# ytgui/SPT-proto

Measured on NVIDIA B200. Metric: sparse_mha_fwd_bwd_tokens_per_s, higher is better.
Workload: dtype bf16

## Files before the change

### spt_proto_b200/csrc/attn_common.cuh

```cuda
#pragma once
#include <cstdlib>
#include <cstring>

#include "tc.cuh"

namespace spt {
namespace attn_tc {

using namespace tc;

constexpr int BM = 128;
constexpr int BN = 64;
constexpr int STAGES = 3;
constexpr int N_MATH = 256;
constexpr int THREADS = 320;
template <int D>
struct Dim {
    static_assert(D == 64 || D == 128, "head dim must be 64 or 128");
    static constexpr int NSUB = D / 64;
    static constexpr int OWN_SUB = BM * 64 * 2, T_SUB = BN * 64 * 2;
    static constexpr int OWN_BYTES = NSUB * OWN_SUB, T_BYTES = NSUB * T_SUB;
    static constexpr int TMEM_COLS = D == 64 ? 256 : 512;
    static constexpr int CTAS = D == 64 ? 2 : 1;
    static constexpr int FWD_SMEM = OWN_BYTES + 2 * STAGES * T_BYTES + 1024  + 1024  + 256 ;
// ... 221 lines not shown
                d0, d1);
            if (CLAMP) {
                d0 = in0 ? d0 : 0.0f;
                d1 = in1 ? d1 : 0.0f;
            }
            pe[i >> 1] = pack_bf16(e0, e1) & m;
            pd[i >> 1] = pack_bf16(d0, d1) & m;
        }
    }
}

#ifdef SPT_ATTN_PROF
static __device__ unsigned long long g_prof[3][16];
struct Prof {
    long long t[8] = {0, 0, 0, 0, 0, 0, 0, 0};
    long long last;
    __device__ __forceinline__ void start() { last = clock64(); }
    __device__ __forceinline__ void lap(int slot) {
        const long long now = clock64();
        t[slot] += now - last;
        last = now;
    }
    __device__ __forceinline__ void flush(int kernel, int base, bool on) {
        if (on)
            for (int i = 0; i < 8; ++i) atomicAdd(&g_prof[kernel][base + i], (unsigned long long)t[i]);
    }
};
#define PROF(...) __VA_ARGS__
#else
#define PROF(...)
#endif

struct Smem {
    uint32_t base;
    unsigned char *ptr;
};
__device__ __forceinline__ Smem align_smem(unsigned char *raw) {
    const uint32_t a = smem_u32(raw);
    const uint32_t base = (a + 1023) & ~1023u;
    return {base, raw + (base - a)};
}
__device__ __forceinline__ void math_warps_sync() { asm volatile("bar.sync 1, %0;" ::"n"(N_MATH) : "memory"); }

__device__ __forceinline__ void store_row32(__nv_bfloat16 *dst, const uint32_t (&r)[32], float s) {
#pragma unroll
    for (int i = 0; i < 32; i += 8) {
        float t[8];
#pragma unroll
        for (int u = 0; u < 8; ++u) t[u] = __uint_as_float(r[i + u]) * s;
        Vec16<__nv_bfloat16>::store(dst + i, t);
    }
}

}

namespace attn_tc128 {
int launch_bwd_kv128(const CUtensorMap &mq, const CUtensorMap &mk, const CUtensorMap &mv, const CUtensorMap &md,
                     const uint32_t *mask, const int32_t *extra0, const float *ndelta, __nv_bfloat16 *gk,
                     __nv_bfloat16 *gv, int B, int S, int H, float scale, float clamp, cudaStream_t st);
int launch_bwd_q128(const CUtensorMap &mq, const CUtensorMap &mk, const CUtensorMap &mv, const CUtensorMap &md,
                    const uint32_t *mask, const int32_t *extra0, const float *ndelta, __nv_bfloat16 *gq, int B, int S,
                    int H, float scale, float clamp, cudaStream_t st);
int launch_bwd_fused128(const CUtensorMap &mq, const CUtensorMap &mk, const CUtensorMap &mv, const CUtensorMap &md,
                        const uint32_t *mask, const int32_t *extra0, const float *ndelta, float *dq_acc,
                        __nv_bfloat16 *gq, __nv_bfloat16 *gk, __nv_bfloat16 *gv, int B, int S, int H, float scale,
                        float clamp, cudaStream_t st);
int launch_fwd128(const CUtensorMap &mq, const CUtensorMap &mk, const CUtensorMap &mv, const uint32_t *mask,
                  const int32_t *extra0, __nv_bfloat16 *y, float *zsum, int B, int S, int H, float scale, float clamp,
                  int y_transposed, cudaStream_t st);
int read_prof(unsigned long long *out48, int reset);
}
}
```

### spt_proto_b200/csrc/attn_tc.cu

```cuda
#include <mutex>

#include "attn_common.cuh"

namespace spt {
namespace attn_tc {


template <int D>
__global__ void __launch_bounds__(THREADS, Dim<D>::CTAS)
attn_fwd_tc_kernel(const __grid_constant__ CUtensorMap map_q, const __grid_constant__ CUtensorMap map_k,
                   const __grid_constant__ CUtensorMap map_v, const uint32_t *__restrict__ mask,
                   const int32_t *__restrict__ extra0, __nv_bfloat16 *__restrict__ y, float *__restrict__ zsum, int S,
                   int H, float scale_log2, float clamp_log2, int y_transposed) {
    constexpr int OWN_BYTES = Dim<D>::OWN_BYTES, T_BYTES = Dim<D>::T_BYTES, OWN_SUB = Dim<D>::OWN_SUB, T_SUB = Dim<D>::T_SUB,
                  TMEM_COLS = Dim<D>::TMEM_COLS;
    constexpr int NBUF = 3;
    extern __shared__ unsigned char smem_raw[];
    const Smem sm = align_smem(smem_raw);
    const uint32_t s_q = sm.base, s_k = s_q + OWN_BYTES, s_v = s_k + STAGES * T_BYTES;
    float *s_part = reinterpret_cast<float *>(sm.ptr + OWN_BYTES + 2 * STAGES * T_BYTES);
    uint64_t *bars = reinterpret_cast<uint64_t *>(sm.ptr + OWN_BYTES + 2 * STAGES * T_BYTES + 1024);
    const uint32_t bar0 = smem_u32(bars);
    const uint32_t q_full = bar0, o_full = bar0 + 8;
    auto k_full = [&](int s) { return bar0 + 16 + s * 8; };
// ... 587 lines not shown
            const bool clamp = warp_needs_clamp(r, mk.thr);
            uint32_t pe[8], pd[8];
#define SPT_KV_HALF(OFF)                                                                                                   \
            if (key0) {                                                                                                    \
                if (clamp) bwdkv_chunk16<true, true, OFF, 32>(r, g, mrow, s_ndelta, s_ex0, c0 + OFF, shl, mk, pe, pd);     \
                else bwdkv_chunk16<true, false, OFF, 32>(r, g, mrow, s_ndelta, s_ex0, c0 + OFF, shl, mk, pe, pd);          \
            } else {                                                                                                       \
                if (clamp) bwdkv_chunk16<false, true, OFF, 32>(r, g, mrow, s_ndelta, s_ex0, c0 + OFF, shl, mk, pe, pd);    \
                else bwdkv_chunk16<false, false, OFF, 32>(r, g, mrow, s_ndelta, s_ex0, c0 + OFF, shl, mk, pe, pd);         \
            }                                                                                                              \
            tmem_st8(col + (OFF) / 2, pe);                          \
            tmem_st8(col + 32 + (OFF) / 2, pd);
            SPT_KV_HALF(0)
            SPT_KV_HALF(16)
#undef SPT_KV_HALF
            PROF(pf.lap(2);)
            tmem_st_wait();
            fence_before_sync();
            mbar_arrive(p_full(h));
            PROF(pf.lap(3);)
        }
        PROF(pf.t[5] = clock64() - t0; pf.t[4] = n_tiles; pf.flush(2, 0, threadIdx.x == 0);)
        mbar_wait(acc_full, 0);
        fence_after_sync();
        const size_t off = (((size_t)hn * S + n0 + kk) * H + hh) * D + half * (D / 2);
#pragma unroll
        for (int c = 0; c < D / 64; ++c) {
            uint32_t r[32];
            tmem_ld32(lane_base + COL_DV + half * (D / 2) + c * 32, r);
            store_row32(dv + off + c * 32, r, 1.0f);
            tmem_ld32(lane_base + COL_DK + half * (D / 2) + c * 32, r);
            store_row32(dk + off + c * 32, r, scale);
        }
    }
    fence_before_sync();
    __syncthreads();
    if (warp == 9) tmem_dealloc<TMEM_COLS>(tmem_base);
}

static int make_map(CUtensorMap *map, const void *base, int N, int S, int H, int D) {
    EncodeTiledFn fn = encode_fn();
    if (!fn) return fail(SPT_ERR_CUDA, "sparse_attn: cuTensorMapEncodeTiled entry point not available");
    cuuint64_t dims[4] = {(cuuint64_t)D, (cuuint64_t)H, (cuuint64_t)S, (cuuint64_t)N};
    cuuint64_t strides[3] = {(cuuint64_t)D * 2, (cuuint64_t)H * D * 2, (cuuint64_t)S * H * D * 2};
    cuuint32_t box[4] = {64, 1, (cuuint32_t)BN, 1};
    cuuint32_t estr[4] = {1, 1, 1, 1};
    CUresult r = fn(map, CU_TENSOR_MAP_DATA_TYPE_BFLOAT16, 4, const_cast<void *>(base), dims, strides, box, estr,
                    CU_TENSOR_MAP_INTERLEAVE_NONE, CU_TENSOR_MAP_SWIZZLE_128B, CU_TENSOR_MAP_L2_PROMOTION_L2_256B,
                    CU_TENSOR_MAP_FLOAT_OOB_FILL_NONE);
    if (r != CUDA_SUCCESS) return fail(SPT_ERR_CUDA, "sparse_attn: cuTensorMapEncodeTiled failed (%d)", (int)r);
    return SPT_OK;
}

static bool tile128() {
    static const bool on = [] { const char *e = getenv("SPT_ATTN_TILE"); return !(e && atoi(e) == 64); }();
    return on;
}
static bool bwd_fused() {
    static const bool on = [] { const char *e = getenv("SPT_ATTN_BWD_FUSED"); return e && atoi(e) == 1; }();
    return on;
}
static bool bwd_two_streams() {
    static const bool on = [] { const char *e = getenv("SPT_ATTN_BWD_STREAMS"); return !(e && atoi(e) == 0); }();
    return on;
}
struct SideStream {
    cudaStream_t stream = nullptr;
    cudaEvent_t fork = nullptr, join = nullptr;
};
static std::mutex g_side_mu;
static SideStream *side_stream(cudaStream_t caller) {
    static SideStream table[64];
    int dev = 0;
    if (cudaGetDevice(&dev) != cudaSuccess || dev < 0 || dev >= 64) return nullptr;
    SideStream &s = table[dev];
    if (!s.stream) {
        cudaStreamCaptureStatus cap = cudaStreamCaptureStatusNone;
        if (cudaStreamIsCapturing(caller, &cap) != cudaSuccess || cap != cudaStreamCaptureStatusNone) return nullptr;
        if (cudaStreamCreateWithFlags(&s.stream, cudaStreamNonBlocking) != cudaSuccess) return nullptr;
        if (cudaEventCreateWithFlags(&s.fork, cudaEventDisableTiming) != cudaSuccess ||
            cudaEventCreateWithFlags(&s.join, cudaEventDisableTiming) != cudaSuccess) {
            s.stream = nullptr;
            return nullptr;
        }
    }
    return &s;
}
static bool fwd128() {
    static const bool on = [] { const char *e = getenv("SPT_ATTN_FWD128"); return e && atoi(e) == 1; }();
    return on;
}

template <int D>
static int launch_fwd(const CUtensorMap &mq, const CUtensorMap &mk, const CUtensorMap &mv, const uint32_t *mask,
                      const int32_t *extra0, __nv_bfloat16 *y, float *zsum, int B, int S, int H, float scale, float clamp,
                      int y_transposed, cudaStream_t st) {
    if (D == 64 && fwd128()) return attn_tc128::launch_fwd128(mq, mk, mv, mask, extra0, y, zsum, B, S, H, scale, clamp, y_transposed, st);
    static const int extra_smem = [] { const char *e = getenv("SPT_ATTN_EXTRA_SMEM"); return e ? atoi(e) : 0; }();
    cudaFuncSetAttribute(attn_fwd_tc_kernel<D>, cudaFuncAttributeMaxDynamicSharedMemorySize, Dim<D>::FWD_SMEM + extra_smem);
    attn_fwd_tc_kernel<D><<<dim3(B, S / BM), THREADS, Dim<D>::FWD_SMEM + extra_smem, st>>>(mq, mk, mv, mask, extra0, y, zsum, S, H,
                                                                              scale * LOG2E, clamp * LOG2E, y_transposed);
    return after_launch("attn_fwd_tc_kernel");
}

template <int D>
static int launch_prep(const __nv_bfloat16 *y, const __nv_bfloat16 *grad_y, const float *zsum, float *delta,
// ... 146 lines not shown
```

### spt_proto_b200/csrc/attn_tc128.cu

```cuda
#include "attn_common.cuh"

namespace spt {
namespace attn_tc128 {

using namespace tc;
using namespace attn_tc;

constexpr int T = 128;
constexpr int MATH_WARPS = 16;
constexpr int THREADS = (MATH_WARPS + 2) * 32;
constexpr int W_TMA = MATH_WARPS, W_MMA = MATH_WARPS + 1;
constexpr int D = 64;
constexpr int TILE = T * D * 2;
constexpr int ST = 3;

__device__ __forceinline__ int sched_item(int round, int n_items) {
    const int G = gridDim.x;
#ifdef SPT_SCHED_PLAIN
    const int item = round * G + (int)blockIdx.x;
#else
    const int item = round * G + ((round & 1) ? G - 1 - (int)blockIdx.x : (int)blockIdx.x);
#endif
    return item < n_items ? item : -1;
}

__device__ __forceinline__ void warp_arrive(uint32_t bar, int lane) {
    fence_before_sync();
    __syncwarp();
    if (lane == 0) mbar_arrive(bar);
}


constexpr int MT = T + 4;
constexpr int ROWQ = MT * 16 + T * 4 + T * 4;
constexpr int KV_SMEM = 4 * TILE + 2 * ST * TILE + ST * ROWQ + 256 + 1024;

__global__ void __launch_bounds__(THREADS, 1)
attn_bwd_kv128_kernel(const __grid_constant__ CUtensorMap map_q, const __grid_constant__ CUtensorMap map_k,
                      const __grid_constant__ CUtensorMap map_v, const __grid_constant__ CUtensorMap map_dys,
                      const uint32_t *__restrict__ mask, const int32_t *__restrict__ extra0,
                      const float *__restrict__ ndelta, __nv_bfloat16 *__restrict__ dk, __nv_bfloat16 *__restrict__ dv,
                      int S, int H, int B, float scale, float scale_log2, float clamp_log2) {
    extern __shared__ unsigned char smem_raw[];
    const Smem sm = align_smem(smem_raw);
    const uint32_t s_k = sm.base, s_v = s_k + 2 * TILE, s_q = s_v + 2 * TILE, s_dy = s_q + ST * TILE;
    unsigned char *rowq = sm.ptr + 4 * TILE + 2 * ST * TILE;
    uint64_t *bars = reinterpret_cast<uint64_t *>(rowq + ST * ROWQ);
    const uint32_t bar0 = smem_u32(bars);
    auto own_full = [&](int i) { return bar0 + i * 8; };
    auto own_empty = [&](int i) { return bar0 + 16 + i * 8; };
    auto qd_full = [&](int s) { return bar0 + 32 + s * 8; };
    auto qd_empty = [&](int s) { return bar0 + 32 + (ST + s) * 8; };
    const uint32_t sc_full = bar0 + 32 + 2 * ST * 8, s_read = sc_full + 8, p_full = sc_full + 16, e_free = sc_full + 24,
                   acc_full = sc_full + 32, acc_empty = sc_full + 40;
    uint32_t *tmem_slot = reinterpret_cast<uint32_t *>(bars + 4 + 2 * ST + 6);

    const int warp = threadIdx.x >> 5, lane = threadIdx.x & 31;
    const int n_own = S / T;
    const int n_items = n_own * B;
    const int words = S / 32;

    if (threadIdx.x == 0) {
        for (int i = 0; i < 2; ++i) {
            mbar_init(own_full(i), 1);
            mbar_init(own_empty(i), 1);
        }
        for (int s = 0; s < ST; ++s) {
            mbar_init(qd_full(s), 2);
            mbar_init(qd_empty(s), 1);
        }
        mbar_init(sc_full, 1);
        mbar_init(s_read, MATH_WARPS);
        mbar_init(p_full, MATH_WARPS);
        mbar_init(e_free, 1);
        mbar_init(acc_full, 1);
        mbar_init(acc_empty, MATH_WARPS);
        mbar_fence_init();
    }
    if (warp == W_MMA) tmem_alloc<512>(smem_u32(tmem_slot));
    fence_before_sync();
    __syncthreads();
    fence_after_sync();
    const uint32_t tmem_base = *tmem_slot;
    constexpr uint32_t COL_S = 0, COL_DP = 128, COL_E = 256, COL_DS = 320, COL_DV = 384, COL_DK = 448;

    if (warp == W_TMA) {
        int g = 0, w = 0;
        for (int item; (item = sched_item(w, n_items)) >= 0; ++w) {
            const int kt = item / B, b = item % B;
            const int hn = b / H, hh = b % H, n0 = kt * T, n_tiles = n_own - kt;
            const size_t head = (size_t)b * S;
            const int buf = w & 1;
            if (lane == 0) {
                mbar_wait(own_empty(buf), ((w >> 1) & 1) ^ 1);
                mbar_expect_tx(own_full(buf), 2 * TILE);
                tma_owner<D>(s_k + buf * TILE, &map_k, own_full(buf), hh, n0, hn);
                tma_owner<D>(s_v + buf * TILE, &map_v, own_full(buf), hh, n0, hn);
            }
            uint4 mw[4];
#pragma unroll
            for (int u = 0; u < 4; ++u)
                mw[u] = __ldg(reinterpret_cast<const uint4 *>(mask + (head + n0 + lane + 32 * u) * words) + kt);
            for (int j = 0; j < n_tiles; ++j, ++g) {
                const int st = g % ST;
                const int r0 = (kt + j) * T;
                unsigned char *slot = rowq + st * ROWQ;
                mbar_wait(qd_empty(st), ((g / ST) & 1) ^ 1);
                if (lane == 0) {
                    mbar_expect_tx(qd_full(st), 2 * TILE + 2 * T * 4);
                    tma_owner<D>(s_q + st * TILE, &map_q, qd_full(st), hh, r0, hn);
                    tma_owner<D>(s_dy + st * TILE, &map_dys, qd_full(st), hh, r0, hn);
                    bulk_load_1d(smem_u32(slot + MT * 16), ndelta + head + r0, T * 4, qd_full(st));
                    bulk_load_1d(smem_u32(slot + MT * 16 + T * 4), extra0 + head + r0, T * 4, qd_full(st));
                }
                uint32_t *mt = reinterpret_cast<uint32_t *>(slot);
#pragma unroll
                for (int u = 0; u < 4; ++u) {
                    const int rr = lane + 32 * u;
                    mt[rr] = mw[u].x;
                    mt[MT + rr] = mw[u].y;
                    mt[2 * MT + rr] = mw[u].z;
                    mt[3 * MT + rr] = mw[u].w;
                }
                if (j + 1 < n_tiles) {
#pragma unroll
                    for (int u = 0; u < 4; ++u)
                        mw[u] = __ldg(reinterpret_cast<const uint4 *>(mask + (head + r0 + T + lane + 32 * u) * words) + kt);
                }
                __syncwarp();
                if (lane == 0) mbar_arrive(qd_full(st));
            }
        }
    } else if (warp == W_MMA) {
        constexpr uint32_t id_s = idesc_bf16(T, T, 0, 0);
        constexpr uint32_t id_a = idesc_bf16(T, D, 0, 1);
        const uint64_t dk0 = desc_kmajor(s_k, 0), dv0 = desc_kmajor(s_v, 0), dq0 = desc_kmajor(s_q, 0),
                       ddy0 = desc_kmajor(s_dy, 0), dqt0 = desc_mnmajor(s_q, 0, TILE), ddyt0 = desc_mnmajor(s_dy, 0, TILE);
        int g = 0, w = 0;
        PROF(Prof pf; pf.start(); const long long t0 = pf.last;)
        for (int item; (item = sched_item(w, n_items)) >= 0; ++w) {
            const int kt = item / B, n_tiles = n_own - kt;
            const int buf = w & 1;
            const uint64_t own_off = (uint64_t)((buf * TILE) >> 4);
            auto issue_scores = [&](int gg) {
                const int st = gg % ST;
                mbar_wait(qd_full(st), (gg / ST) & 1);
                if (gg > 0) mbar_wait(s_read, (gg - 1) & 1);
                fence_after_sync();
                if (elect_one()) {
                    const uint64_t off = (uint64_t)((st * TILE) >> 4);
#pragma unroll
                    for (int k = 0; k < D / 16; ++k) {
                        umma_bf16(tmem_base + COL_S, dk0 + own_off + k * KMAJOR_K16, dq0 + off + k * KMAJOR_K16, id_s, k != 0);
                        umma_bf16(tmem_base + COL_DP, dv0 + own_off + k * KMAJOR_K16, ddy0 + off + k * KMAJOR_K16, id_s, k != 0);
                    }
                    umma_commit(sc_full);
                }
                __syncwarp();
            };
            mbar_wait(own_full(buf), (w >> 1) & 1);
            issue_scores(g);
            for (int j = 0; j < n_tiles; ++j, ++g) {
                PROF(pf.lap(2);)
                if (j + 1 < n_tiles) issue_scores(g + 1);
                PROF(pf.lap(0);)
                const int st = g % ST;
                mbar_wait(p_full, g & 1);
                if (j == 0 && w > 0) mbar_wait(acc_empty, (w - 1) & 1);
                PROF(pf.lap(1);)
                fence_after_sync();
                if (elect_one()) {
                    const uint64_t off = (uint64_t)((st * TILE) >> 4);
#pragma unroll
                    for (int k = 0; k < T / 16; ++k) {
                        umma_bf16_ts(tmem_base + COL_DV, tmem_base + COL_E + k * 8, ddyt0 + off + k * MNMAJOR_K16, id_a, (j | k) != 0);
                        umma_bf16_ts(tmem_base + COL_DK, tmem_base + COL_DS + k * 8, dqt0 + off + k * MNMAJOR_K16, id_a, (j | k) != 0);
                    }
                    umma_commit(qd_empty(st));
                    umma_commit(e_free);
                    if (j + 1 == n_tiles) {
                        umma_commit(acc_full);
                        umma_commit(own_empty(buf));
                    }
                }
                __syncwarp();
            }
        }
        PROF(pf.t[3] = clock64() - t0; pf.t[4] = g; pf.flush(2, 8, lane == 0);)
    } else {
        const int quarter = warp & 3, cg = warp >> 2;
        const int kk = quarter * 32 + lane;
        const int wsel = kk & 3;
        const int shl = 31 - (kk >> 2);
        const MathK mk = make_math(scale_log2, clamp_log2);
        const uint32_t lane_base = tmem_base + ((uint32_t)(quarter * 32) << 16);
        const int c0 = cg * 32;
        int g = 0, w = 0;
        PROF(Prof pf; pf.start(); const long long t0 = pf.last;)
        for (int item; (item = sched_item(w, n_items)) >= 0; ++w) {
            const int kt = item / B, b = item % B;
            const int hn = b / H, hh = b % H, n0 = kt * T, n_tiles = n_own - kt;
            const bool key0 = (n0 + kk) == 0;
            for (int j = 0; j < n_tiles; ++j, ++g) {
                const int st = g % ST;
                const unsigned char *slot = rowq + st * ROWQ;
                const uint32_t *mrow = reinterpret_cast<const uint32_t *>(slot) + wsel * MT;
                const float *s_nd = reinterpret_cast<const float *>(slot + MT * 16);
                const int32_t *s_ex0 = reinterpret_cast<const int32_t *>(slot + MT * 16 + T * 4);
                mbar_wait(qd_full(st), (g / ST) & 1);
                mbar_wait(sc_full, g & 1);
                PROF(pf.lap(0);)
                fence_after_sync();
                uint32_t r[32], gr[32];
                tmem_ld32_nowait(lane_base + COL_S + c0, r);
                tmem_ld32_nowait(lane_base + COL_DP + c0, gr);
                tmem_ld_wait();
                warp_arrive(s_read, lane);
                PROF(pf.lap(1);)
                const bool clamp = warp_needs_clamp(r, mk.thr);
                bool pad = false;
                if (key0) {
#pragma unroll
                    for (int i = 0; i < 32; i += 4) {
                        const int4 e4 = *reinterpret_cast<const int4 *>(s_ex0 + c0 + i);
                        pad |= (e4.x | e4.y | e4.z | e4.w) != 0;
                    }
                }
                uint32_t pe0[8], pd0[8], pe1[8], pd1[8];
#define SPT_KV_HALF(OFF, PE, PD)                                                                                           \
                if (pad) {                                                                                                \
                    if (clamp) bwdkv_chunk16<true, true, OFF, 32>(r, gr, mrow, s_nd, s_ex0, c0 + OFF, shl, mk, PE, PD);    \
                    else bwdkv_chunk16<true, false, OFF, 32>(r, gr, mrow, s_nd, s_ex0, c0 + OFF, shl, mk, PE, PD);         \
                } else {                                                                                                   \
                    if (clamp) bwdkv_chunk16<false, true, OFF, 32>(r, gr, mrow, s_nd, s_ex0, c0 + OFF, shl, mk, PE, PD);   \
                    else bwdkv_chunk16<false, false, OFF, 32>(r, gr, mrow, s_nd, s_ex0, c0 + OFF, shl, mk, PE, PD);        \
                }
                SPT_KV_HALF(0, pe0, pd0)
                SPT_KV_HALF(16, pe1, pd1)
#undef SPT_KV_HALF
                PROF(pf.lap(2);)
                if (g > 0) {
                    mbar_wait(e_free, (g - 1) & 1);
                    fence_after_sync();
                }
                tmem_st8(lane_base + COL_E + c0 / 2, pe0);
                tmem_st8(lane_base + COL_E + c0 / 2 + 8, pe1);
                tmem_st8(lane_base + COL_DS + c0 / 2, pd0);
                tmem_st8(lane_base + COL_DS + c0 / 2 + 8, pd1);
                tmem_st_wait();
                warp_arrive(p_full, lane);
                PROF(pf.lap(3);)
            }
            mbar_wait(acc_full, w & 1);
            fence_after_sync();
            {
                uint32_t o[32];
                tmem_ld32(lane_base + COL_DV + c0, o);
                warp_arrive(acc_empty, lane);
                const size_t off = (((size_t)hn * S + n0 + kk) * H + hh) * D + (cg & 1) * 32;
                store_row32((cg < 2 ? dv : dk) + off, o, cg < 2 ? 1.0f : scale);
            }
            PROF(pf.lap(5);)
        }
        PROF(pf.t[6] = clock64() - t0; pf.t[4] = g; pf.flush(2, 0, threadIdx.x == 0);)
    }
    fence_before_sync();
    __syncthreads();
    if (warp == W_MMA) tmem_dealloc<512>(tmem_base);
}

int launch_bwd_kv128(const CUtensorMap &mq, const CUtensorMap &mk, const CUtensorMap &mv, const CUtensorMap &md,
                     const uint32_t *mask, const int32_t *extra0, const float *ndelta, __nv_bfloat16 *gk,
                     __nv_bfloat16 *gv, int B, int S, int H, float scale, float clamp, cudaStream_t st) {
    cudaFuncSetAttribute(attn_bwd_kv128_kernel, cudaFuncAttributeMaxDynamicSharedMemorySize, KV_SMEM);
    const int n_items = (S / T) * B;
    const int grid = n_items < num_sms() ? n_items : num_sms();
    attn_bwd_kv128_kernel<<<grid, THREADS, KV_SMEM, st>>>(mq, mk, mv, md, mask, extra0, ndelta, gk, gv, S, H, B, scale,
                                                        scale * LOG2E, clamp * LOG2E);
    return after_launch("attn_bwd_kv128_kernel");
}


__device__ __forceinline__ void store_row16(__nv_bfloat16 *dst, const uint32_t (&r)[16], float s) {
#pragma unroll
    for (int i = 0; i < 16; i += 8) {
        float t[8];
#pragma unroll
        for (int u = 0; u < 8; ++u) t[u] = __uint_as_float(r[i + u]) * s;
        Vec16<__nv_bfloat16>::store(dst + i, t);
    }
}
__device__ __forceinline__ void tmem_ld16(uint32_t taddr, uint32_t (&r)[16]) {
    tmem_ld16_nowait(taddr, r);
    tmem_ld_wait();
}
__device__ __forceinline__ void math_sync() { asm volatile("bar.sync 1, %0;" ::"n"(MATH_WARPS * 32) : "memory"); }

constexpr int FUSED_SMEM = 3 * TILE + 2 * ST * TILE + 2 * TILE + 2 * TILE + ST * ROWQ + 256 + 1024;
static_assert(FUSED_SMEM <= 227 * 1024, "fused backward: shared memory budget");

__global__ void __launch_bounds__(THREADS, 1)
attn_bwd_fused128_kernel(const __grid_constant__ CUtensorMap map_q, const __grid_constant__ CUtensorMap map_k,
                         const __grid_constant__ CUtensorMap map_v, const __grid_constant__ CUtensorMap map_dys,
                         const uint32_t *__restrict__ mask, const int32_t *__restrict__ extra0,
                         const float *__restrict__ ndelta, float *__restrict__ dq_acc, __nv_bfloat16 *__restrict__ dk,
                         __nv_bfloat16 *__restrict__ dv, int S, int H, int B, float scale, float scale_log2,
                         float clamp_log2) {
    extern __shared__ unsigned char smem_raw[];
    const Smem sm = align_smem(smem_raw);
    const uint32_t s_k = sm.base, s_v = s_k + 2 * TILE, s_q = s_v + TILE, s_dy = s_q + ST * TILE, s_ds = s_dy + ST * TILE,
                   s_st = s_ds + 2 * TILE;
    unsigned char *rowq = sm.ptr + (7 + 2 * ST) * TILE;
    uint64_t *bars = reinterpret_cast<uint64_t *>(rowq + ST * ROWQ);
    const uint32_t bar0 = smem_u32(bars);
    auto own_full = [&](int i) { return bar0 + i * 8; };
    auto own_empty = [&](int i) { return bar0 + 16 + i * 8; };
    auto qd_full = [&](int s) { return bar0 + 32 + s * 8; };
    auto qd_empty = [&](int s) { return bar0 + 32 + (ST + s) * 8; };
    const uint32_t sc_full = bar0 + 32 + 2 * ST * 8, s_read = sc_full + 8, p_full = sc_full + 16, e_free = sc_full + 24,
                   acc_full = sc_full + 32, acc_empty = sc_full + 40, v_full = sc_full + 48, v_empty = sc_full + 56,
                   dq_empty = sc_full + 64;
    uint32_t *tmem_slot = reinterpret_cast<uint32_t *>(bars + 4 + 2 * ST + 9);

    const int warp = threadIdx.x >> 5, lane = threadIdx.x & 31;
    const int n_own = S / T;
    const int n_items = n_own * B;
    const int words = S / 32;

    if (threadIdx.x == 0) {
        for (int i = 0; i < 2; ++i) {
// ... 321 lines not shown
    const int warp = threadIdx.x >> 5, lane = threadIdx.x & 31;
    const int n_own = S / T;
    const int n_items = n_own * B;

    if (threadIdx.x == 0) {
        for (int i = 0; i < 2; ++i) {
            mbar_init(own_full(i), 1);
            mbar_init(own_empty(i), 1);
            mbar_init(p_full(i), MATH_WARPS);
            mbar_init(e_free(i), 1);
        }
        for (int s = 0; s < ST; ++s) {
            mbar_init(kv_full(s), 1);
            mbar_init(kv_empty(s), 1);
        }
        mbar_init(sc_full, 1);
        mbar_init(s_read, MATH_WARPS);
        mbar_init(acc_full, 1);
        mbar_init(acc_empty, MATH_WARPS);
        mbar_fence_init();
    }
    if (warp == W_MMA) tmem_alloc<512>(smem_u32(tmem_slot));
    fence_before_sync();
    __syncthreads();
    fence_after_sync();
    const uint32_t tmem_base = *tmem_slot;
    constexpr uint32_t COL_S = 0, COL_DP = 128, COL_DS = 256, COL_DQ = 384;

    if (warp == W_TMA) {
        if (lane == 0) {
            int g = 0, w = 0;
            for (int item; (item = sched_item(w, n_items)) >= 0; ++w) {
                const int qt = n_own - 1 - item / B, b = item % B;
                const int hn = b / H, hh = b % H, n_tiles = qt + 1;
                const int buf = w & 1;
                mbar_wait(own_empty(buf), ((w >> 1) & 1) ^ 1);
                mbar_expect_tx(own_full(buf), 2 * TILE);
                tma_owner<D>(s_q + buf * TILE, &map_q, own_full(buf), hh, qt * T, hn);
                tma_owner<D>(s_dy + buf * TILE, &map_dys, own_full(buf), hh, qt * T, hn);
                for (int j = 0; j < n_tiles; ++j, ++g) {
                    const int st = g % ST;
                    mbar_wait(kv_empty(st), ((g / ST) & 1) ^ 1);
                    mbar_expect_tx(kv_full(st), 2 * TILE);
                    tma_owner<D>(s_k + st * TILE, &map_k, kv_full(st), hh, j * T, hn);
                    tma_owner<D>(s_v + st * TILE, &map_v, kv_full(st), hh, j * T, hn);
                }
            }
        }
    } else if (warp == W_MMA) {
        constexpr uint32_t id_s = idesc_bf16(T, T, 0, 0);
        constexpr uint32_t id_a = idesc_bf16(T, D, 0, 1);
        const uint64_t dq0 = desc_kmajor(s_q, 0), ddy0 = desc_kmajor(s_dy, 0), dk0 = desc_kmajor(s_k, 0),
                       dv0 = desc_kmajor(s_v, 0), dkt0 = desc_mnmajor(s_k, 0, TILE);
        int g = 0, w = 0;
        PROF(Prof pf; pf.start(); const long long t0 = pf.last;)
        for (int item; (item = sched_item(w, n_items)) >= 0; ++w) {
            const int n_tiles = n_own - item / B;
            const int buf = w & 1;
            const uint64_t own_off = (uint64_t)((buf * TILE) >> 4);
            auto issue_scores = [&](int gg) {
                const int st = gg % ST;
                mbar_wait(kv_full(st), (gg / ST) & 1);
                if (gg > 0) mbar_wait(s_read, (gg - 1) & 1);
                fence_after_sync();
                if (elect_one()) {
                    const uint64_t off = (uint64_t)((st * TILE) >> 4);
#pragma unroll
                    for (int k = 0; k < D / 16; ++k) {
                        umma_bf16(tmem_base + COL_S, dq0 + own_off + k * KMAJOR_K16, dk0 + off + k * KMAJOR_K16, id_s, k != 0);
                        umma_bf16(tmem_base + COL_DP, ddy0 + own_off + k * KMAJOR_K16, dv0 + off + k * KMAJOR_K16, id_s, k != 0);
                    }
                    umma_commit(sc_full);
                }
                __syncwarp();
            };
            mbar_wait(own_full(buf), (w >> 1) & 1);
            issue_scores(g);
            for (int j = 0; j < n_tiles; ++j, ++g) {
                PROF(pf.lap(2);)
                if (j + 1 < n_tiles) issue_scores(g + 1);
                PROF(pf.lap(0);)
                const int st = g % ST;
                mbar_wait(p_full(g & 1), (g >> 1) & 1);
                if (j == 0 && w > 0) mbar_wait(acc_empty, (w - 1) & 1);
                PROF(pf.lap(1);)
                fence_after_sync();
                if (elect_one()) {
                    const uint64_t off = (uint64_t)((st * TILE) >> 4);
#pragma unroll
                    for (int k = 0; k < T / 16; ++k)
                        umma_bf16_ts(tmem_base + COL_DQ, tmem_base + COL_DS + (g & 1) * 64 + k * 8, dkt0 + off + k * MNMAJOR_K16, id_a,
                                     (j | k) != 0);
                    umma_commit(kv_empty(st));
                    umma_commit(e_free(g & 1));
                    if (j + 1 == n_tiles) {
                        umma_commit(acc_full);
                        umma_commit(own_empty(buf));
                    }
                }
                __syncwarp();
            }
        }
        PROF(pf.t[3] = clock64() - t0; pf.t[4] = g; pf.flush(1, 8, lane == 0);)
    } else {
        const int quarter = warp & 3, cg = warp >> 2;
        const int rt = quarter * 32 + lane;
        const MathK mk = make_math(scale_log2, clamp_log2);
        const uint32_t lane_base = tmem_base + ((uint32_t)(quarter * 32) << 16);
        int g = 0, w = 0;
        PROF(Prof pf; pf.start(); const long long t0 = pf.last;)
        for (int item; (item = sched_item(w, n_items)) >= 0; ++w) {
            const int qt = n_own - 1 - item / B, b = item % B;
            const int hn = b / H, hh = b % H, n_tiles = qt + 1;
            const int row = qt * T + rt;
            const size_t grow = (size_t)b * S + row;
            const uint4 *mrow = reinterpret_cast<const uint4 *>(mask + grow * (S / 32));
            const float ex0 = (float)extra0[grow];
            const float nd = ndelta[grow];
            uint4 mw = __ldg(mrow);
            for (int j = 0; j < n_tiles; ++j, ++g) {
                const uint4 mw_next = (j + 1 < n_tiles) ? __ldg(mrow + j + 1) : mw;
                mbar_wait(sc_full, g & 1);
                PROF(pf.lap(0);)
                fence_after_sync();
                uint32_t r[32], gr[32];
                tmem_ld32_nowait(lane_base + COL_S + cg * 32, r);
                tmem_ld32_nowait(lane_base + COL_DP + cg * 32, gr);
                tmem_ld_wait();
                warp_arrive(s_read, lane);
                PROF(pf.lap(1);)
                const uint32_t X = chunk_mask_bytes(mw, cg);
                uint32_t pk[16];
                const bool first = (j == 0 && cg == 0);
                if (!warp_needs_clamp(r, mk.thr)) {
                    if (first) bwdq_chunk32<true, false>(r, gr, X, mk, nd, ex0, pk);
                    else bwdq_chunk32<false, false>(r, gr, X, mk, nd, ex0, pk);
                } else {
                    if (first) bwdq_chunk32<true, true>(r, gr, X, mk, nd, ex0, pk);
                    else bwdq_chunk32<false, true>(r, gr, X, mk, nd, ex0, pk);
                }
                PROF(pf.lap(2);)
                if (g >= 2) {
                    mbar_wait(e_free(g & 1), ((g >> 1) - 1) & 1);
                    fence_after_sync();
                }
                tmem_st16(lane_base + COL_DS + (g & 1) * 64 + cg * 16, pk);
                tmem_st_wait();
                warp_arrive(p_full(g & 1), lane);
                PROF(pf.lap(3);)
                mw = mw_next;
            }
            mbar_wait(acc_full, w & 1);
            fence_after_sync();
            {
                uint32_t o[16];
                tmem_ld16(lane_base + COL_DQ + cg * 16, o);
                warp_arrive(acc_empty, lane);
                store_row16(dq + (((size_t)hn * S + row) * H + hh) * D + cg * 16, o, scale);
            }
            PROF(pf.lap(5);)
        }
        PROF(pf.t[6] = clock64() - t0; pf.t[4] = g; pf.flush(1, 0, threadIdx.x == 0);)
    }
    fence_before_sync();
    __syncthreads();
    if (warp == W_MMA) tmem_dealloc<512>(tmem_base);
}

constexpr int F_SMEM = 2 * TILE + 2 * ST * TILE + 4 * T * 4 + 256 + 1024;

__global__ void __launch_bounds__(THREADS, 1)
attn_fwd128_kernel(const __grid_constant__ CUtensorMap map_q, const __grid_constant__ CUtensorMap map_k,
                   const __grid_constant__ CUtensorMap map_v, const uint32_t *__restrict__ mask,
                   const int32_t *__restrict__ extra0, __nv_bfloat16 *__restrict__ y, float *__restrict__ zsum, int S,
                   int H, int B, float scale_log2, float clamp_log2, int y_transposed) {
    extern __shared__ unsigned char smem_raw[];
    const Smem sm = align_smem(smem_raw);
    const uint32_t s_q = sm.base, s_k = s_q + 2 * TILE, s_v = s_k + ST * TILE;
    float *s_part = reinterpret_cast<float *>(sm.ptr + 2 * TILE + 2 * ST * TILE);
    uint64_t *bars = reinterpret_cast<uint64_t *>(sm.ptr + 2 * TILE + 2 * ST * TILE + 4 * T * 4);
    const uint32_t bar0 = smem_u32(bars);
    auto own_full = [&](int i) { return bar0 + i * 8; };
    auto own_empty = [&](int i) { return bar0 + 16 + i * 8; };
    auto k_full = [&](int s) { return bar0 + 32 + s * 8; };
    auto k_empty = [&](int s) { return bar0 + 32 + (ST + s) * 8; };
    auto v_full = [&](int s) { return bar0 + 32 + (2 * ST + s) * 8; };
    auto v_empty = [&](int s) { return bar0 + 32 + (3 * ST + s) * 8; };
    const uint32_t sc_full = bar0 + 32 + 4 * ST * 8, s_read = sc_full + 8, acc_full = sc_full + 16, acc_empty = sc_full + 24;
    auto p_full = [&](int i) { return sc_full + 32 + i * 8; };
    auto e_free = [&](int i) { return sc_full + 48 + i * 8; };
    uint32_t *tmem_slot = reinterpret_cast<uint32_t *>(bars + 4 + 4 * ST + 8);

    const int warp = threadIdx.x >> 5, lane = threadIdx.x & 31;
    const int n_own = S / T;
    const int n_items = n_own * B;

    if (threadIdx.x == 0) {
        for (int i = 0; i < 2; ++i) {
            mbar_init(own_full(i), 1);
            mbar_init(own_empty(i), 1);
            mbar_init(p_full(i), MATH_WARPS);
            mbar_init(e_free(i), 1);
        }
        for (int s = 0; s < ST; ++s) {
            mbar_init(k_full(s), 1);
            mbar_init(k_empty(s), 1);
            mbar_init(v_full(s), 1);
            mbar_init(v_empty(s), 1);
        }
        mbar_init(sc_full, 1);
        mbar_init(s_read, MATH_WARPS);
        mbar_init(acc_full, 1);
        mbar_init(acc_empty, MATH_WARPS);
        mbar_fence_init();
    }
// ... 200 lines not shown
```

Measured before the change: 12.39 million.

## Pipeline backward attention across work items and TMA-load mask tiles

In the dK/dV and dQ backward kernels, the MMA warp now issues the first scores MMA of the next work item before finishing the current one. The math warps defer the previous item's accumulator epilogue until after the first tile of the next item, so the tile-boundary bubble is overlapped. The dK/dV kernel also loads mask blocks with a 2D TMA into a staged buffer and transposes them one step behind, replacing per-lane __ldg loads on the producer warp. This costs extra shared memory, more barriers and more complex phase tracking.

```diff
diff --git a/spt_proto_b200/csrc/attn_common.cuh b/spt_proto_b200/csrc/attn_common.cuh
--- a/spt_proto_b200/csrc/attn_common.cuh
+++ b/spt_proto_b200/csrc/attn_common.cuh
@@ -297,6 +297,8 @@
     }
 }
 
+int make_mask_map(CUtensorMap *map, const uint32_t *mask, int B, int S);
+
 }
 
 namespace attn_tc128 {
diff --git a/spt_proto_b200/csrc/attn_tc.cu b/spt_proto_b200/csrc/attn_tc.cu
--- a/spt_proto_b200/csrc/attn_tc.cu
+++ b/spt_proto_b200/csrc/attn_tc.cu
@@ -663,6 +663,20 @@
     return SPT_OK;
 }
 
+int make_mask_map(CUtensorMap *map, const uint32_t *mask, int B, int S) {
+    EncodeTiledFn fn = encode_fn();
+    if (!fn) return fail(SPT_ERR_CUDA, "sparse_attn: cuTensorMapEncodeTiled entry point not available");
+    cuuint64_t dims[2] = {(cuuint64_t)S / 32, (cuuint64_t)B * S};
+    cuuint64_t strides[1] = {(cuuint64_t)S / 8};
+    cuuint32_t box[2] = {4, 128};
+    cuuint32_t estr[2] = {1, 1};
+    CUresult r = fn(map, CU_TENSOR_MAP_DATA_TYPE_UINT32, 2, const_cast<uint32_t *>(mask), dims, strides, box, estr,
+                    CU_TENSOR_MAP_INTERLEAVE_NONE, CU_TENSOR_MAP_SWIZZLE_NONE, CU_TENSOR_MAP_L2_PROMOTION_NONE,
+                    CU_TENSOR_MAP_FLOAT_OOB_FILL_NONE);
+    if (r != CUDA_SUCCESS) return fail(SPT_ERR_CUDA, "sparse_attn: cuTensorMapEncodeTiled (mask) failed (%d)", (int)r);
+    return SPT_OK;
+}
+
 static bool tile128() {
     static const bool on = [] { const char *e = getenv("SPT_ATTN_TILE"); return !(e && atoi(e) == 64); }();
     return on;
diff --git a/spt_proto_b200/csrc/attn_tc128.cu b/spt_proto_b200/csrc/attn_tc128.cu
--- a/spt_proto_b200/csrc/attn_tc128.cu
+++ b/spt_proto_b200/csrc/attn_tc128.cu
@@ -33,32 +33,36 @@
 
 constexpr int MT = T + 4;
 constexpr int ROWQ = MT * 16 + T * 4 + T * 4;
-constexpr int KV_SMEM = 4 * TILE + 2 * ST * TILE + ST * ROWQ + 256 + 1024;
+constexpr int MBOX = T * 16;
+constexpr int KV_SMEM = 4 * TILE + 2 * ST * TILE + ST * (MBOX + ROWQ) + 256 + 1024;
+static_assert(KV_SMEM <= 227 * 1024, "dK/dV backward: shared memory budget");
 
 __global__ void __launch_bounds__(THREADS, 1)
 attn_bwd_kv128_kernel(const __grid_constant__ CUtensorMap map_q, const __grid_constant__ CUtensorMap map_k,
                       const __grid_constant__ CUtensorMap map_v, const __grid_constant__ CUtensorMap map_dys,
-                      const uint32_t *__restrict__ mask, const int32_t *__restrict__ extra0,
+                      const __grid_constant__ CUtensorMap map_mask, const int32_t *__restrict__ extra0,
                       const float *__restrict__ ndelta, __nv_bfloat16 *__restrict__ dk, __nv_bfloat16 *__restrict__ dv,
                       int S, int H, int B, float scale, float scale_log2, float clamp_log2) {
     extern __shared__ unsigned char smem_raw[];
     const Smem sm = align_smem(smem_raw);
     const uint32_t s_k = sm.base, s_v = s_k + 2 * TILE, s_q = s_v + 2 * TILE, s_dy = s_q + ST * TILE;
-    unsigned char *rowq = sm.ptr + 4 * TILE + 2 * ST * TILE;
+    unsigned char *mbox = sm.ptr + 4 * TILE + 2 * ST * TILE;
+    unsigned char *rowq = mbox + ST * MBOX;
     uint64_t *bars = reinterpret_cast<uint64_t *>(rowq + ST * ROWQ);
     const uint32_t bar0 = smem_u32(bars);
     auto own_full = [&](int i) { return bar0 + i * 8; };
     auto own_empty = [&](int i) { return bar0 + 16 + i * 8; };
     auto qd_full = [&](int s) { return bar0 + 32 + s * 8; };
     auto qd_empty = [&](int s) { return bar0 + 32 + (ST + s) * 8; };
-    const uint32_t sc_full = bar0 + 32 + 2 * ST * 8, s_read = sc_full + 8, p_full = sc_full + 16, e_free = sc_full + 24,
+    auto m_land = [&](int s) { return bar0 + 32 + (2 * ST + s) * 8; };
+    auto m_full = [&](int s) { return bar0 + 32 + (3 * ST + s) * 8; };
+    const uint32_t sc_full = bar0 + 32 + 4 * ST * 8, s_read = sc_full + 8, p_full = sc_full + 16, e_free = sc_full + 24,
                    acc_full = sc_full + 32, acc_empty = sc_full + 40;
-    uint32_t *tmem_slot = reinterpret_cast<uint32_t *>(bars + 4 + 2 * ST + 6);
+    uint32_t *tmem_slot = reinterpret_cast<uint32_t *>(bars + 4 + 4 * ST + 6);
 
     const int warp = threadIdx.x >> 5, lane = threadIdx.x & 31;
     const int n_own = S / T;
     const int n_items = n_own * B;
-    const int words = S / 32;
 
     if (threadIdx.x == 0) {
         for (int i = 0; i < 2; ++i) {
@@ -66,8 +70,10 @@
             mbar_init(own_empty(i), 1);
         }
         for (int s = 0; s < ST; ++s) {
-            mbar_init(qd_full(s), 2);
+            mbar_init(qd_full(s), 1);
             mbar_init(qd_empty(s), 1);
+            mbar_init(m_land(s), 1);
+            mbar_init(m_full(s), 1);
         }
         mbar_init(sc_full, 1);
         mbar_init(s_read, MATH_WARPS);
@@ -85,6 +91,25 @@
     constexpr uint32_t COL_S = 0, COL_DP = 128, COL_E = 256, COL_DS = 320, COL_DV = 384, COL_DK = 448;
 
     if (warp == W_TMA) {
+        PROF(Prof pf; pf.start();)
+        auto transpose = [&](int gg) {
+            const int st = gg % ST;
+            mbar_wait(m_land(st), (gg / ST) & 1);
+            const uint4 *box = reinterpret_cast<const uint4 *>(mbox + st * MBOX);
+            uint32_t *mt = reinterpret_cast<uint32_t *>(rowq + st * ROWQ);
+#pragma unroll
+            for (int u = 0; u < 4; ++u) {
+                const int rr = lane + 32 * u;
+                const uint4 m = box[rr];
+                mt[rr] = m.x;
+                mt[MT + rr] = m.y;
+                mt[2 * MT + rr] = m.z;
+                mt[3 * MT + rr] = m.w;
+            }
+            __syncwarp();
+            if (lane == 0) mbar_arrive(m_full(st));
+            PROF(pf.lap(7);)
+        };
         int g = 0, w = 0;
         for (int item; (item = sched_item(w, n_items)) >= 0; ++w) {
             const int kt = item / B, b = item % B;
@@ -97,77 +122,72 @@
                 tma_owner<D>(s_k + buf * TILE, &map_k, own_full(buf), hh, n0, hn);
                 tma_owner<D>(s_v + buf * TILE, &map_v, own_full(buf), hh, n0, hn);
             }
-            uint4 mw[4];
-#pragma unroll
-            for (int u = 0; u < 4; ++u)
-                mw[u] = __ldg(reinterpret_cast<const uint4 *>(mask + (head + n0 + lane + 32 * u) * words) + kt);
             for (int j = 0; j < n_tiles; ++j, ++g) {
                 const int st = g % ST;
                 const int r0 = (kt + j) * T;
                 unsigned char *slot = rowq + st * ROWQ;
                 mbar_wait(qd_empty(st), ((g / ST) & 1) ^ 1);
+                PROF(pf.lap(6);)
                 if (lane == 0) {
                     mbar_expect_tx(qd_full(st), 2 * TILE + 2 * T * 4);
                     tma_owner<D>(s_q + st * TILE, &map_q, qd_full(st), hh, r0, hn);
                     tma_owner<D>(s_dy + st * TILE, &map_dys, qd_full(st), hh, r0, hn);
                     bulk_load_1d(smem_u32(slot + MT * 16), ndelta + head + r0, T * 4, qd_full(st));
                     bulk_load_1d(smem_u32(slot + MT * 16 + T * 4), extra0 + head + r0, T * 4, qd_full(st));
-                }
-                uint32_t *mt = reinterpret_cast<uint32_t *>(slot);
-#pragma unroll
-                for (int u = 0; u < 4; ++u) {
-                    const int rr = lane + 32 * u;
-                    mt[rr] = mw[u].x;
-                    mt[MT + rr] = mw[u].y;
-                    mt[2 * MT + rr] = mw[u].z;
-                    mt[3 * MT + rr] = mw[u].w;
-                }
-                if (j + 1 < n_tiles) {
-#pragma unroll
-                    for (int u = 0; u < 4; ++u)
-                        mw[u] = __ldg(reinterpret_cast<const uint4 *>(mask + (head + r0 + T + lane + 32 * u) * words) + kt);
+                    mbar_expect_tx(m_land(st), MBOX);
+                    tma_load_2d(smem_u32(mbox + st * MBOX), &map_mask, m_land(st), kt * 4, (int)(head + r0));
                 }
                 __syncwarp();
-                if (lane == 0) mbar_arrive(qd_full(st));
-            }
-        }
+                if (g > 0) transpose(g - 1);
+            }
+        }
+        if (g > 0) transpose(g - 1);
+        PROF(pf.flush(2, 8, lane == 0);)
     } else if (warp == W_MMA) {
         constexpr uint32_t id_s = idesc_bf16(T, T, 0, 0);
         constexpr uint32_t id_a = idesc_bf16(T, D, 0, 1);
         const uint64_t dk0 = desc_kmajor(s_k, 0), dv0 = desc_kmajor(s_v, 0), dq0 = desc_kmajor(s_q, 0),
                        ddy0 = desc_kmajor(s_dy, 0), dqt0 = desc_mnmajor(s_q, 0, TILE), ddyt0 = desc_mnmajor(s_dy, 0, TILE);
+        auto issue_scores = [&](int gg, int bb) {
+            const int st = gg % ST;
+            mbar_wait(qd_full(st), (gg / ST) & 1);
+            if (gg > 0) mbar_wait(s_read, (gg - 1) & 1);
+            fence_after_sync();
+            if (elect_one()) {
+                const uint64_t off = (uint64_t)((st * TILE) >> 4), own_off = (uint64_t)((bb * TILE) >> 4);
+#pragma unroll
+                for (int k = 0; k < D / 16; ++k) {
+                    umma_bf16(tmem_base + COL_S, dk0 + own_off + k * KMAJOR_K16, dq0 + off + k * KMAJOR_K16, id_s, k != 0);
+                    umma_bf16(tmem_base + COL_DP, dv0 + own_off + k * KMAJOR_K16, ddy0 + off + k * KMAJOR_K16, id_s, k != 0);
+                }
+                umma_commit(sc_full);
+            }
+            __syncwarp();
+        };
         int g = 0, w = 0;
         PROF(Prof pf; pf.start(); const long long t0 = pf.last;)
-        for (int item; (item = sched_item(w, n_items)) >= 0; ++w) {
+        int item = sched_item(0, n_items);
+        if (item >= 0) {
+            mbar_wait(own_full(0), 0);
+            issue_scores(0, 0);
+        }
+        for (; item >= 0; ++w) {
+            const int next = sched_item(w + 1, n_items);
             const int kt = item / B, n_tiles = n_own - kt;
             const int buf = w & 1;
-            const uint64_t own_off = (uint64_t)((buf * TILE) >> 4);
-            auto issue_scores = [&](int gg) {
-                const int st = gg % ST;
-                mbar_wait(qd_full(st), (gg / ST) & 1);
-                if (gg > 0) mbar_wait(s_read, (gg - 1) & 1);
-                fence_after_sync();
-                if (elect_one()) {
-                    const uint64_t off = (uint64_t)((st * TILE) >> 4);
-#pragma unroll
-                    for (int k = 0; k < D / 16; ++k) {
-                        umma_bf16(tmem_base + COL_S, dk0 + own_off + k * KMAJOR_K16, dq0 + off + k * KMAJOR_K16, id_s, k != 0);
-                        umma_bf16(tmem_base + COL_DP, dv0 + own_off + k * KMAJOR_K16, ddy0 + off + k * KMAJOR_K16, id_s, k != 0);
-                    }
-                    umma_commit(sc_full);
-                }
-                __syncwarp();
-            };
-            mbar_wait(own_full(buf), (w >> 1) & 1);
-            issue_scores(g);
             for (int j = 0; j < n_tiles; ++j, ++g) {
-                PROF(pf.lap(2);)
-                if (j + 1 < n_tiles) issue_scores(g + 1);
+                PROF(pf.lap(j == 0 && w > 0 ? 5 : 2);)
+                if (j + 1 < n_tiles) {
+                    issue_scores(g + 1, buf);
+                } else if (next >= 0) {
+                    mbar_wait(own_full(buf ^ 1), ((w + 1) >> 1) & 1);
+                    issue_scores(g + 1, buf ^ 1);
+                }
                 PROF(pf.lap(0);)
                 const int st = g % ST;
                 mbar_wait(p_full, g & 1);
                 if (j == 0 && w > 0) mbar_wait(acc_empty, (w - 1) & 1);
-                PROF(pf.lap(1);)
+                PROF(pf.lap(j == 0 && w > 0 ? 5 : 1);)
                 fence_after_sync();
                 if (elect_one()) {
                     const uint64_t off = (uint64_t)((st * TILE) >> 4);
@@ -185,6 +205,7 @@
                 }
                 __syncwarp();
             }
+            item = next;
         }
         PROF(pf.t[3] = clock64() - t0; pf.t[4] = g; pf.flush(2, 8, lane == 0);)
     } else {
@@ -195,7 +216,17 @@
         const MathK mk = make_math(scale_log2, clamp_log2);
         const uint32_t lane_base = tmem_base + ((uint32_t)(quarter * 32) << 16);
         const int c0 = cg * 32;
+        auto epilogue = [&](int ww, int e_hn, int e_hh, int e_n0) {
+            mbar_wait(acc_full, ww & 1);
+            fence_after_sync();
+            uint32_t o[32];
+            tmem_ld32(lane_base + COL_DV + c0, o);
+            warp_arrive(acc_empty, lane);
+            const size_t off = (((size_t)e_hn * S + e_n0 + kk) * H + e_hh) * D + (cg & 1) * 32;
+            store_row32((cg < 2 ? dv : dk) + off, o, cg < 2 ? 1.0f : scale);
+        };
         int g = 0, w = 0;
+        int p_hn = 0, p_hh = 0, p_n0 = 0;
         PROF(Prof pf; pf.start(); const long long t0 = pf.last;)
         for (int item; (item = sched_item(w, n_items)) >= 0; ++w) {
             const int kt = item / B, b = item % B;
@@ -208,8 +239,9 @@
                 const float *s_nd = reinterpret_cast<const float *>(slot + MT * 16);
                 const int32_t *s_ex0 = reinterpret_cast<const int32_t *>(slot + MT * 16 + T * 4);
                 mbar_wait(qd_full(st), (g / ST) & 1);
+                mbar_wait(m_full(st), (g / ST) & 1);
                 mbar_wait(sc_full, g & 1);
-                PROF(pf.lap(0);)
+                PROF(pf.lap(j == 0 && w > 0 ? 5 : 0);)
                 fence_after_sync();
                 uint32_t r[32], gr[32];
                 tmem_ld32_nowait(lane_base + COL_S + c0, r);
@@ -243,26 +275,25 @@
                     mbar_wait(e_free, (g - 1) & 1);
                     fence_after_sync();
                 }
+                PROF(pf.lap(3);)
                 tmem_st8(lane_base + COL_E + c0 / 2, pe0);
                 tmem_st8(lane_base + COL_E + c0 / 2 + 8, pe1);
                 tmem_st8(lane_base + COL_DS + c0 / 2, pd0);
                 tmem_st8(lane_base + COL_DS + c0 / 2 + 8, pd1);
                 tmem_st_wait();
                 warp_arrive(p_full, lane);
-                PROF(pf.lap(3);)
-            }
-            mbar_wait(acc_full, w & 1);
-            fence_after_sync();
-            {
-                uint32_t o[32];
-                tmem_ld32(lane_base + COL_DV + c0, o);
-                warp_arrive(acc_empty, lane);
-                const size_t off = (((size_t)hn * S + n0 + kk) * H + hh) * D + (cg & 1) * 32;
-                store_row32((cg < 2 ? dv : dk) + off, o, cg < 2 ? 1.0f : scale);
-            }
-            PROF(pf.lap(5);)
-        }
-        PROF(pf.t[6] = clock64() - t0; pf.t[4] = g; pf.flush(2, 0, threadIdx.x == 0);)
+                PROF(pf.lap(7);)
+                if (j == 0 && w > 0) {
+                    epilogue(w - 1, p_hn, p_hh, p_n0);
+                    PROF(pf.lap(5);)
+                }
+            }
+            p_hn = hn;
+            p_hh = hh;
+            p_n0 = n0;
+        }
+        if (w > 0) epilogue(w - 1, p_hn, p_hh, p_n0);
+        PROF(pf.lap(5); pf.t[6] = clock64() - t0; pf.t[4] = g; pf.flush(2, 0, threadIdx.x == 0);)
     }
     fence_before_sync();
     __syncthreads();
@@ -272,10 +303,13 @@
 int launch_bwd_kv128(const CUtensorMap &mq, const CUtensorMap &mk, const CUtensorMap &mv, const CUtensorMap &md,
                      const uint32_t *mask, const int32_t *extra0, const float *ndelta, __nv_bfloat16 *gk,
                      __nv_bfloat16 *gv, int B, int S, int H, float scale, float clamp, cudaStream_t st) {
+    CUtensorMap mm;
+    const int rc = make_mask_map(&mm, mask, B, S);
+    if (rc != SPT_OK) return rc;
     cudaFuncSetAttribute(attn_bwd_kv128_kernel, cudaFuncAttributeMaxDynamicSharedMemorySize, KV_SMEM);
     const int n_items = (S / T) * B;
     const int grid = n_items < num_sms() ? n_items : num_sms();
-    attn_bwd_kv128_kernel<<<grid, THREADS, KV_SMEM, st>>>(mq, mk, mv, md, mask, extra0, ndelta, gk, gv, S, H, B, scale,
+    attn_bwd_kv128_kernel<<<grid, THREADS, KV_SMEM, st>>>(mq, mk, mv, md, mm, extra0, ndelta, gk, gv, S, H, B, scale,
                                                         scale * LOG2E, clamp * LOG2E);
     return after_launch("attn_bwd_kv128_kernel");
 }
@@ -703,38 +737,46 @@
         constexpr uint32_t id_a = idesc_bf16(T, D, 0, 1);
         const uint64_t dq0 = desc_kmajor(s_q, 0), ddy0 = desc_kmajor(s_dy, 0), dk0 = desc_kmajor(s_k, 0),
                        dv0 = desc_kmajor(s_v, 0), dkt0 = desc_mnmajor(s_k, 0, TILE);
+        auto issue_scores = [&](int gg, int bb) {
+            const int st = gg % ST;
+            mbar_wait(kv_full(st), (gg / ST) & 1);
+            if (gg > 0) mbar_wait(s_read, (gg - 1) & 1);
+            fence_after_sync();
+            if (elect_one()) {
+                const uint64_t off = (uint64_t)((st * TILE) >> 4), own_off = (uint64_t)((bb * TILE) >> 4);
+#pragma unroll
+                for (int k = 0; k < D / 16; ++k) {
+                    umma_bf16(tmem_base + COL_S, dq0 + own_off + k * KMAJOR_K16, dk0 + off + k * KMAJOR_K16, id_s, k != 0);
+                    umma_bf16(tmem_base + COL_DP, ddy0 + own_off + k * KMAJOR_K16, dv0 + off + k * KMAJOR_K16, id_s, k != 0);
+                }
+                umma_commit(sc_full);
+            }
+            __syncwarp();
+        };
         int g = 0, w = 0;
         PROF(Prof pf; pf.start(); const long long t0 = pf.last;)
-        for (int item; (item = sched_item(w, n_items)) >= 0; ++w) {
+        int item = sched_item(0, n_items);
+        if (item >= 0) {
+            mbar_wait(own_full(0), 0);
+            issue_scores(0, 0);
+        }
+        for (; item >= 0; ++w) {
+            const int next = sched_item(w + 1, n_items);
             const int n_tiles = n_own - item / B;
             const int buf = w & 1;
-            const uint64_t own_off = (uint64_t)((buf * TILE) >> 4);
-            auto issue_scores = [&](int gg) {
-                const int st = gg % ST;
-                mbar_wait(kv_full(st), (gg / ST) & 1);
-                if (gg > 0) mbar_wait(s_read, (gg - 1) & 1);
-                fence_after_sync();
-                if (elect_one()) {
-                    const uint64_t off = (uint64_t)((st * TILE) >> 4);
-#pragma unroll
-                    for (int k = 0; k < D / 16; ++k) {
-                        umma_bf16(tmem_base + COL_S, dq0 + own_off + k * KMAJOR_K16, dk0 + off + k * KMAJOR_K16, id_s, k != 0);
-                        umma_bf16(tmem_base + COL_DP, ddy0 + own_off + k * KMAJOR_K16, dv0 + off + k * KMAJOR_K16, id_s, k != 0);
-                    }
-                    umma_commit(sc_full);
-                }
-                __syncwarp();
-            };
-            mbar_wait(own_full(buf), (w >> 1) & 1);
-            issue_scores(g);
             for (int j = 0; j < n_tiles; ++j, ++g) {
-                PROF(pf.lap(2);)
-                if (j + 1 < n_tiles) issue_scores(g + 1);
+                PROF(pf.lap(j == 0 && w > 0 ? 5 : 2);)
+                if (j + 1 < n_tiles) {
+                    issue_scores(g + 1, buf);
+                } else if (next >= 0) {
+                    mbar_wait(own_full(buf ^ 1), ((w + 1) >> 1) & 1);
+                    issue_scores(g + 1, buf ^ 1);
+                }
                 PROF(pf.lap(0);)
                 const int st = g % ST;
                 mbar_wait(p_full(g & 1), (g >> 1) & 1);
                 if (j == 0 && w > 0) mbar_wait(acc_empty, (w - 1) & 1);
-                PROF(pf.lap(1);)
+                PROF(pf.lap(j == 0 && w > 0 ? 5 : 1);)
                 fence_after_sync();
                 if (elect_one()) {
                     const uint64_t off = (uint64_t)((st * TILE) >> 4);
@@ -751,6 +793,7 @@
                 }
                 __syncwarp();
             }
+            item = next;
         }
         PROF(pf.t[3] = clock64() - t0; pf.t[4] = g; pf.flush(1, 8, lane == 0);)
     } else {
@@ -758,7 +801,16 @@
         const int rt = quarter * 32 + lane;
         const MathK mk = make_math(scale_log2, clamp_log2);
         const uint32_t lane_base = tmem_base + ((uint32_t)(quarter * 32) << 16);
+        auto epilogue = [&](int ww, int e_hn, int e_hh, int e_row) {
+            mbar_wait(acc_full, ww & 1);
+            fence_after_sync();
+            uint32_t o[16];
+            tmem_ld16(lane_base + COL_DQ + cg * 16, o);
+            warp_arrive(acc_empty, lane);
+            store_row16(dq + (((size_t)e_hn * S + e_row) * H + e_hh) * D + cg * 16, o, scale);
+        };
         int g = 0, w = 0;
+        int p_hn = 0, p_hh = 0, p_row = 0;
         PROF(Prof pf; pf.start(); const long long t0 = pf.last;)
         for (int item; (item = sched_item(w, n_items)) >= 0; ++w) {
             const int qt = n_own - 1 - item / B, b = item % B;
@@ -772,7 +824,7 @@
             for (int j = 0; j < n_tiles; ++j, ++g) {
                 const uint4 mw_next = (j + 1 < n_tiles) ? __ldg(mrow + j + 1) : mw;
                 mbar_wait(sc_full, g & 1);
-                PROF(pf.lap(0);)
+                PROF(pf.lap(j == 0 && w > 0 ? 5 : 0);)
                 fence_after_sync();
                 uint32_t r[32], gr[32];
                 tmem_ld32_nowait(lane_base + COL_S + cg * 32, r);
@@ -795,23 +847,23 @@
                     mbar_wait(e_free(g & 1), ((g >> 1) - 1) & 1);
                     fence_after_sync();
                 }
+                PROF(pf.lap(3);)
                 tmem_st16(lane_base + COL_DS + (g & 1) * 64 + cg * 16, pk);
                 tmem_st_wait();
                 warp_arrive(p_full(g & 1), lane);
-                PROF(pf.lap(3);)
+                PROF(pf.lap(7);)
                 mw = mw_next;
-            }
-            mbar_wait(acc_full, w & 1);
-            fence_after_sync();
-            {
-                uint32_t o[16];
-                tmem_ld16(lane_base + COL_DQ + cg * 16, o);
-                warp_arrive(acc_empty, lane);
-                store_row16(dq + (((size_t)hn * S + row) * H + hh) * D + cg * 16, o, scale);
-            }
-            PROF(pf.lap(5);)
-        }
-        PROF(pf.t[6] = clock64() - t0; pf.t[4] = g; pf.flush(1, 0, threadIdx.x == 0);)
+                if (j == 0 && w > 0) {
+                    epilogue(w - 1, p_hn, p_hh, p_row);
+                    PROF(pf.lap(5);)
+                }
+            }
+            p_hn = hn;
+            p_hh = hh;
+            p_row = row;
+        }
+        if (w > 0) epilogue(w - 1, p_hn, p_hh, p_row);
+        PROF(pf.lap(5); pf.t[6] = clock64() - t0; pf.t[4] = g; pf.flush(1, 0, threadIdx.x == 0);)
     }
     fence_before_sync();
     __syncthreads();
```

After: 12.50 million, median of 6. About the same (+0.9%).
